# wouter-rombouts/fast-losless-image-compression-format

Measured on AMD Instinct MI355X. Metric: encode+decode MPixels/s on 4K RGBA at 1/2/4/8 MI355X; bitstream bit-exact, higher is better.
Workload: dtype u8

## Files before the change

fast-losless-image-compression-format_amd/csrc/nice_capi.hip:

```cpp
#include <hip/hip_runtime.h>
#include <stdint.h>
#include <stdio.h>
#include <stdlib.h>
#include <string.h>

#include <atomic>
#include <cmath>
#include <mutex>
#include <algorithm>
#include <vector>

#include "../../include/nice.h"
#include "../../include/nice_test.h"
#include "nice_format.h"
#include "nice_bits.hpp"
#include "nice_kernels.h"
#include "nice_dec_plan.hpp"
#include "nice_enc_plan.hpp"
#include "nice_slot_plan.hpp"
#include "nice_rec.hpp"
#include "nice_resize.hpp"
#include "nice_tiles.hpp"
#include "nice_internal.h"

// ... 400 lines not shown
  tm.end(st);
  tm.begin(NICE_PH_ENC_HEADER, st);
  hipLaunchKernelGGL(enc_header, grid_of(P.header), dim3(P.header.threads), 0, st, a);
  tm.end(st);
  if (T > 0) {
    tm.begin(NICE_PH_ENC_TILEBITS, st);
    hipLaunchKernelGGL(enc_packtab, grid_of(P.packtab), dim3(P.packtab.threads), 0, st, a);
    tm.end(st);
    launch_pack(P, a, st, &tm);
    tm.begin(NICE_PH_ENC_TAIL, st);
    hipLaunchKernelGGL(enc_tail, grid_of(P.tail), dim3(P.tail.threads), 0, st, a);
    tm.end(st);
  }
  NICE_HIP(hipGetLastError());
  return NICE_OK;
}


namespace {
struct DecLayout {
  size_t total;
  size_t o_tables, o_dstart, o_entry, o_last, o_ck, o_cpx, o_cstart, o_recs, o_changed, o_fchanged, o_rowbuf;
  size_t o_ev, o_evck, o_evn, o_agree, o_items, o_icount;
  size_t o_hand, o_abort;
};
constexpr uint32_t kSyncQueuedMax = 16, kSyncFlags = kSyncQueuedMax + 2;
constexpr uint32_t kSettledFlag = kSyncQueuedMax, kFinalFlag = kSyncQueuedMax + 1;
#ifndef NICE_SYNC_QUEUED
#define NICE_SYNC_QUEUED 8
#endif
constexpr uint32_t kSyncQueued = NICE_SYNC_QUEUED;
static_assert(kSyncQueued >= 1 && kSyncQueued <= kSyncQueuedMax, "queued sync iterations");
DecLayout dec_layout(uint32_t n_frames, uint64_t npx, const DecPlan& p) {
  const uint32_t max_chunks = p.max_chunks, n_ck = p.n_ck, ev_cap = p.ev_cap, subs = p.subs;
  DecLayout L{};
  size_t o = 0;
  auto take = [&](size_t bytes) { size_t r = o; o = align_up(o + bytes, 256); return r; };
  L.o_tables = take((size_t)n_frames * sizeof(DecTables));
  L.o_dstart = take((size_t)n_frames * 8);
  L.o_entry = take((size_t)n_frames * max_chunks * 8);
  L.o_last = take((size_t)n_frames * max_chunks * 8);
  L.o_ck = take((size_t)n_frames * n_ck * max_chunks * 8);
  L.o_cpx = take((size_t)n_frames * max_chunks * 8);
  L.o_cstart = take((size_t)n_frames * max_chunks * 8);
  L.o_recs = take((size_t)n_frames * ((npx + 3) & ~3ull) * 4);
  L.o_changed = take(4 * kSyncFlags);
  L.o_fchanged = take((size_t)n_frames * 4);
  L.o_rowbuf = take(p.rowbuf);
  L.o_ev = take((size_t)n_frames * ((max_chunks + 63) & ~63u) * ev_cap * 4);
  L.o_evck = take(ev_cap ? (size_t)n_frames * n_ck * max_chunks * 4 : 0);
  L.o_evn = take(ev_cap ? (size_t)n_frames * max_chunks * 4 : 0);
  L.o_agree = take(ev_cap ? (size_t)n_frames * max_chunks * 4 : 0);
  L.o_items = take(ev_cap ? (size_t)n_frames * max_chunks * subs * 4 : 0);
  L.o_icount = take(ev_cap ? (size_t)n_frames * 4 : 0);
  L.o_hand = take(p.hand);
  L.o_abort = take(p.abort_flags ? (size_t)n_frames * 4 : 0);
  L.total = o;
  return L;
}

void dec_args_scratch(DecArgs& a, const DecLayout& L, uint8_t* base, const DecPlan& P, uint64_t N) {
  a.tables = base + L.o_tables;
  a.data_start = (unsigned long long*)(base + L.o_dstart);
  const uint32_t max_chunks = P.max_chunks, cb = P.slice_bits;
  a.max_chunks = max_chunks;
  a.chunk_bits = cb;
  a.n_ck = P.n_ck;
  a.ck_bits = P.ck_bits;
  a.emit_blocks = (uint32_t)(((uint64_t)max_chunks * (cb / DEC_EMIT_BITS) + DEC_PARSE_THREADS - 1) / DEC_PARSE_THREADS);
  a.chunk_blocks = (max_chunks + DEC_PARSE_THREADS - 1) / DEC_PARSE_THREADS;
  a.chunk_px = (unsigned long long*)(base + L.o_cpx);
  a.chunk_start = (unsigned long long*)(base + L.o_cstart);
  a.entry = (unsigned long long*)(base + L.o_entry);
  a.last = (unsigned long long*)(base + L.o_last);
  a.ck = (unsigned long long*)(base + L.o_ck);
  a.recs = (uint32_t*)(base + L.o_recs);
  a.rec_stride = (N + 3) & ~3ull;
  a.seg = P.g.seg;
  a.nseg = P.g.nseg;
  a.rows_in_lds = P.g.in_lds ? 1u : 0u;
  a.parse_slow = opt_on(NICE_OPT_DEC_SLOW_PARSE) ? 1u : 0u;
  a.rowbuf = (uint32_t*)(base + L.o_rowbuf);
  if (P.ev_cap) {
    a.ev = (uint32_t*)(base + L.o_ev);
    a.ev_cap = P.ev_cap;
    a.ev_ck = (uint32_t*)(base + L.o_evck);
    a.ev_n = (uint32_t*)(base + L.o_evn);
    a.agree = (uint32_t*)(base + L.o_agree);
    a.head_items = (uint32_t*)(base + L.o_items);
    a.head_count = (uint32_t*)(base + L.o_icount);
  }
}

int launch_rows(const DecPlan& p, const DecLaunch& l, DecArgs& a, hipStream_t st) {
  void (*k)(DecArgs) = nullptr;
  switch (l.route) {
    case DEC_R_RECONSTRUCT: k = dec_reconstruct; break;
    case DEC_R_ROWS: k = dec_rows; break;
    case DEC_R_ROWS8: k = dec_rows8; break;
    case DEC_R_ROWS_WIDE: k = dec_rows_wide; break;
    case DEC_R_FLOW: k = dec_rows_flow; break;
    case DEC_R_SPLIT: k = dec_rows_split; break;
    default: return NICE_E_ARG;
  }
  if (l.lds > LDS_OPT_IN)
    NICE_HIP(hipFuncSetAttribute((const void*)k, hipFuncAttributeMaxDynamicSharedMemorySize, (int)l.lds));
  if (l.route != DEC_R_SPLIT) {
    hipLaunchKernelGGL(k, dim3(a.n_frames), dim3(l.threads), l.lds, st, a);
    return NICE_OK;
  }
  for (uint32_t f0 = 0; f0 < a.n_frames; f0 += p.split_frames) {
    a.split_f0 = f0;
    hipLaunchKernelGGL(k, dim3(std::min(p.split_frames, a.n_frames - f0) * p.strips), dim3(l.threads), l.lds, st, a);
// ... 14 lines not shown
          "recomputed_px=%llu fixup_rounds=%llu sync_iters=%u seg=%u nseg=%u "
          "clk[load=%llu spec=%llu fix=%llu emit=%llu]\n",
          h[0], h[1], h[2], h[3], h[4], it_count, a.seg, a.nseg, h[5], h[6], h[7], h[8]);
  fprintf(stderr, "[nice dec stats] sync iterations that changed an entry:");
  for (uint32_t i = 0; i < kSyncFlags; ++i) fprintf(stderr, " %u", chg[i]);
  fprintf(stderr, " (queued %u, then settled, final)\n", queued);
  for (int w = 0; w < 4; ++w) {
    const unsigned long long* q = h + 64 + 8 * w;
    if (q[7])
      fprintf(stderr, "[nice flow stats] wave %d rows=%llu cyc/row: emit+decode=%.0f wait=%.0f ring=%.0f spec=%.0f "
              "fix=%.0f publish=%.0f rounds/row=%.2f\n", w, q[7], (double)q[0] / q[7], (double)q[1] / q[7],
              (double)q[2] / q[7], (double)q[3] / q[7], (double)q[4] / q[7], (double)q[5] / q[7],
              (double)q[6] / q[7]);
  }
  fprintf(stderr, "[nice dec stats] unknown segment tails: copies of an unknown %llu, narrowed %llu\n", h[24], h[25]);
  fprintf(stderr, "[nice dec stats] re-parse met previous parse at checkpoint:");
  for (int k = 0; k < 17; ++k) fprintf(stderr, " %d:%llu", k, h[32 + k]);
  fprintf(stderr, "\n");
  fprintf(stderr, "[nice dec stats] slice=%u emit waves=%llu wave_iters=%llu active_lane_iters=%llu fills=%llu\n",
          a.chunk_bits, h[20], h[16], h[17], h[18]);
  fprintf(stderr, "[nice dec stats] slices by first-pass meeting checkpoint: 0:%llu 1:%llu 2-4:%llu 5-16:%llu "
          "17-64:%llu 65+:%llu none:%llu overflow:%llu (ev_cap %u)\n",
          h[50], h[51], h[52], h[53], h[54], h[55], h[56], h[57], a.ev_cap);
  fprintf(stderr, "[nice dec stats] fix-up rounds per row: 0:%llu 1:%llu 2:%llu 3:%llu 4:%llu 5:%llu 6+:%llu\n",
          h[9], h[10], h[11], h[12], h[13], h[14], h[15]);
  if (h[61]) fprintf(stderr, "[nice dec stats] sync first pass: waves=%llu cycles/wave=%.0f refill cycles/wave=%.0f "
          "refills/wave=%.1f iterations/wave=%.1f active lane share=%.3f\n",
          h[61], h[61] ? (double)h[56] / h[61] : 0.0, h[61] ? (double)h[57] / h[61] : 0.0,
          h[61] ? (double)h[58] / h[61] : 0.0, h[61] ? (double)h[59] / h[61] : 0.0,
          h[59] ? (double)h[60] / (64.0 * h[59]) : 0.0);
}
}

static std::mutex g_default_mu;
static nice_ctx* g_default = nullptr;

static int default_ctx(nice_ctx** out) {
  std::lock_guard<std::mutex> g(g_default_mu);
  if (!g_default) {
    int dev = 0;
    (void)hipGetDevice(&dev);
    int rc = nice_ctx_create(dev, &g_default);
    if (rc) return rc;
  }
  *out = g_default;
  return NICE_OK;
// ... 116 lines not shown
  NICE_HIP(hipSetDevice(ctx->device));
  hipStream_t st = (hipStream_t)stream;
  ctx->split_frames = 0;
  NICE_HIP(hipMemsetAsync(d_status, 0, (size_t)n_frames * 4, st));
  std::vector<uint64_t> lens(n_frames);
  if (h_stream_len) {
    std::copy(h_stream_len, h_stream_len + n_frames, lens.begin());
  } else {
    NICE_HIP(hipMemcpyAsync(lens.data(), d_stream_len, (size_t)n_frames * 8, hipMemcpyDeviceToHost, st));
    NICE_HIP(hipStreamSynchronize(st));
  }
  uint64_t max_len = 0;
  for (uint64_t& l : lens) {
    if (!packed && l > stream_stride) return NICE_E_ARG;
    if (packed && l > packed_bytes) l = 0;
    max_len = l > max_len ? l : max_len;
  }
  const uint64_t D = FILE_HEADER_BYTES * 8 + TABLE_HEADER_BITS;
  uint64_t total_bits = 0;
  for (uint64_t l : lens) total_bits += l * 8 > D ? l * 8 - D : 0;
  auto opt = [](int id) { return DecOpt{opt_set(id), opt_val(id)}; };
  const DecOpts opts{opt(NICE_OPT_DEC_SLICE_BITS), opt(NICE_OPT_DEC_SINGLE_WAVE), opt(NICE_OPT_DEC_SEG),
                     opt(NICE_OPT_DEC_SPLIT),      opt(NICE_OPT_DEC_FLOW),        opt(NICE_OPT_DEC_NO_EVENTS),
                     opt(NICE_OPT_DEC_EV_CAP)};
  DecPlan P = plan_decode(DecShape{n_frames, w, h, ctx->cus, max_len, total_bits}, opts);
  ctx->last_dec_route = P.rows.route;
  ctx->last_dec_fallback = P.fallback.route;
  if (N > 0 && P.rows.route == DEC_R_NONE) return NICE_E_ARG;
  DecLayout L = dec_layout(n_frames, N, P);
  int rc = ctx->dec.grow(L.total);
  if (rc && P.ev_cap) {
    (void)hipGetLastError();
    P.ev_cap = 0;
    L = dec_layout(n_frames, N, P);
    rc = ctx->dec.grow(L.total);
  }
  if (rc) return rc;
  const uint32_t max_chunks = P.max_chunks;
  uint8_t* base = (uint8_t*)ctx->dec.ptr;
  DecArgs a{};
  a.streams = d_streams;
  a.stream_stride = stream_stride;
  a.stream_len = (const unsigned long long*)d_stream_len;
  a.stream_off = (const unsigned long long*)d_stream_off;
  a.packed_bytes = packed_bytes;
  a.n_frames = n_frames;
  a.W = w;
  a.H = h;
  a.out_channels = out_channels;
  a.flags = flags;
  a.px_out = d_px;
  a.px_stride = px_stride;
  a.status = d_status;
// ... 1394 lines not shown
```

fast-losless-image-compression-format_amd/csrc/nice_dec_plan.hpp:

```cpp
#pragma once
#include <stddef.h>
#include <stdint.h>

#include "nice_format.h"
#include "nice_geom.h"

namespace nice {

struct DecShape {
  uint32_t n_frames, w, h;
  int cus;
  uint64_t max_len;
  uint64_t total_bits;
};
struct DecOpt {
  bool set;
  int64_t val;
  bool on() const { return set && val != 0; }
};
struct DecOpts { DecOpt slice_bits, single_wave, seg, split, flow, no_events, ev_cap; };

enum DecRoute : uint32_t { DEC_R_NONE, DEC_R_RECONSTRUCT, DEC_R_ROWS, DEC_R_ROWS8, DEC_R_ROWS_WIDE, DEC_R_FLOW, DEC_R_SPLIT };
constexpr uint32_t dec_route_max_threads(DecRoute r) {
  return r == DEC_R_RECONSTRUCT ? 64 : r == DEC_R_ROWS || r == DEC_R_ROWS8 ? ROWS_THREADS
       : r == DEC_R_ROWS_WIDE ? ROWS_WIDE_THREADS : r == DEC_R_FLOW ? FLOW_THREADS : r == DEC_R_SPLIT ? SPLIT_THREADS : 0;
}
struct DecLaunch {
  DecRoute route;
  uint32_t threads;
  size_t lds;
};
struct RecGeom {
  uint32_t seg, nseg, R;
  size_t lds;
  bool in_lds;
};
struct DecPlan {
  uint32_t slice_bits, max_chunks, ck_bits, n_ck, ev_cap, subs;
  DecLaunch rows;
  DecLaunch fallback;
  uint32_t strips, split_frames;
  uint32_t flow_k, flow_ring;
  size_t rowbuf, hand;
  bool abort_flags;
  RecGeom g;
};

inline RecGeom rec_geom(uint32_t w) {
  auto align4 = [](size_t v) { return (v + 3) / 4 * 4; };
  RecGeom g;
  uint32_t s = (w + DEC_MAX_SEGS - 1) / DEC_MAX_SEGS;
  if (s < 6) s = 6;
  g.seg = s;
  g.nseg = w ? (w + s - 1) / s : 1;
  if (g.nseg > 1 && w - (g.nseg - 1) * s < 6) g.nseg -= 1;
  g.R = w >= 3 ? 4 : 8;
  const size_t kw = (w + 31) / 32;
  const size_t head = 512 + align4(kw) * 4 + align4(w) * 4;
  const size_t ring = (size_t)g.R * w * 4;
  g.in_lds = head + ring <= 150 * 1024;
  g.lds = g.in_lds ? head + ring : head;
  return g;
}

inline DecPlan plan_decode(const DecShape& s, const DecOpts& o) {
  const uint32_t w = s.w, n_frames = s.n_frames;
  DecPlan p{};
  const uint64_t D = FILE_HEADER_BYTES * 8 + TABLE_HEADER_BITS;
  uint32_t cb = s.total_bits >= (48ull << 20) ? 2 * DEC_MIN_CHUNK_BITS : DEC_MIN_CHUNK_BITS;
  while (cb < DEC_MAX_CHUNK_BITS && s.total_bits / (2ull * cb) > 256ull * 8 * 64 * 2) cb *= 2;
  if (o.slice_bits.set) {
    const uint32_t v = (uint32_t)o.slice_bits.val;
    if (v >= DEC_MIN_CHUNK_BITS && v <= DEC_MAX_CHUNK_BITS && (v & (v - 1)) == 0) cb = v;
  }
  p.slice_bits = cb;
  p.max_chunks = s.max_len * 8 > D ? (uint32_t)((s.max_len * 8 - D + cb - 1) / cb) : 1;
  p.ck_bits = cb <= 4096u ? DEC_CK_BITS_SMALL : DEC_CK_BITS;
  p.n_ck = cb / p.ck_bits - 1;
  p.subs = cb / DEC_EMIT_BITS;
  p.ev_cap = o.no_events.on() ? 0u : cb / 4;
  if (o.ev_cap.set) {
    const uint32_t v = (uint32_t)o.ev_cap.val;
    if (p.ev_cap && v >= 4 && v % 4 == 0 && v < p.ev_cap) p.ev_cap = v;
  }
  const RecGeom g = p.g = rec_geom(w);
  const uint32_t cus = (uint32_t)(s.cus > 1 ? s.cus : 1);

  const uint32_t nseg16 = (w + ROWS_SEG - 1) / ROWS_SEG;
  const uint32_t rows_wpr = (nseg16 + 63) / 64, rows_thr = rows_wpr * 64;
  const bool single_wave = o.single_wave.on();
  const bool use_rows = w >= 64 && rows_thr <= ROWS_WIDE_THREADS && !single_wave;
  const size_t rows_lds = rows_lds_bytes(rows_thr, w, true);
  const bool rows_in_lds = rows_thr <= ROWS_THREADS && lds_fits(rows_lds);
  const uint32_t rows8_thr = ((w + 7) / 8 + 63) / 64 * 64;
  const size_t rows8_lds = rows_lds_bytes(rows8_thr, w, true);
  const bool rows8 = o.seg.set && o.seg.val == 8 && use_rows && rows_in_lds && rows8_thr <= ROWS_THREADS &&
                     lds_fits(rows8_lds);
  const uint32_t split_cap = (uint32_t)(s.cus / 2 > 1 ? s.cus / 2 : 1);
  uint32_t strips = (nseg16 + SPLIT_THREADS - 1) / SPLIT_THREADS;
  if (o.split.set) strips = (uint32_t)o.split.val;
  bool split = !single_wave && w >= 64 && strips >= 2 && strips <= split_cap &&
               (!use_rows || (uint64_t)n_frames * strips <= split_cap);
  if (split && !o.split.set && use_rows && w <= FLOW_MAX_W && !o.seg.on() && !(o.flow.set && o.flow.val <= 0))
    split = false;
  const uint32_t sps = split ? (nseg16 + strips - 1) / strips : 0;
  if (split && (sps > SPLIT_THREADS || nseg16 <= (strips - 1) * sps + 1)) split = false;
// ... 47 lines not shown
```

fast-losless-image-compression-format_amd/csrc/nice_decode.hip:

```cpp
#include <hip/hip_runtime.h>
#include <stdint.h>

#include <type_traits>

#include "../../include/nice.h"
#include "nice_bits.hpp"
#include "nice_dec_rec.hpp"
#include "nice_format.h"
#include "nice_kernels.h"

namespace nice {

__device__ __forceinline__ uint32_t n_chunks(uint64_t len, uint64_t D, uint32_t cb) {
  const uint64_t bits = len * 8;
  return bits > D ? (uint32_t)((bits - D + cb - 1) / cb) : 0u;
}

__global__ __launch_bounds__(256) void dec_tables(DecArgs a) {
  __shared__ uint8_t lens[N_BINS];
  __shared__ uint8_t smax[N_STREAMS];
  __shared__ uint16_t order[N_BINS];
  __shared__ int bad;
  const uint32_t f = blockIdx.x;
  const uint64_t len = a.stream_len[f];
// ... 494 lines not shown
  return c > 0xFFFFFFFFull ? 0xFFFFFFFFu : (uint32_t)c;
}
__device__ __forceinline__ uint32_t sat_add(uint32_t a, uint32_t b) { return a + b < a ? 0xFFFFFFFFu : a + b; }

constexpr unsigned long long PS_MASK = (1ull << 51) - 1ull;
__device__ __forceinline__ unsigned long long ps_pack(unsigned long long rel, uint32_t dk) {
  return rel | ((unsigned long long)dk << 44);
}


__global__ __launch_bounds__(256) void dec_init_entries(DecArgs a) {
  const uint32_t f = blockIdx.y;
  for (uint32_t j = blockIdx.x * 256 + threadIdx.x; j < a.max_chunks; j += gridDim.x * 256) {
    const uint64_t i = (uint64_t)f * a.max_chunks + j;
    a.entry[i] = ps_pack((unsigned long long)j * a.chunk_bits, 0);
    a.last[i] = ~0ull;
  }
}

__device__ __forceinline__ uint64_t ev_group(const DecArgs& a, uint32_t f, uint32_t j) {
  return ((uint64_t)f * ((a.max_chunks + 63u) & ~63u) + (j & ~63u)) * a.ev_cap + (j & 63u) * 4u;
}
__device__ __forceinline__ uint32_t ev_word(uint32_t y) { return (y >> 2) * 256u + (y & 3u); }

__device__ __forceinline__ uint32_t ev_pack(uint32_t pfx, uint32_t s0, uint32_t s1, uint32_t s2, uint32_t s3) {
  return pfx | (s0 << 3) | (s1 << 12) | (s2 << 20) | (pfx == (uint32_t)P_LUMA ? s3 << 7 : 0u);
}

__global__ __launch_bounds__(DEC_PARSE_THREADS) PARSE_ATTR void dec_sync(DecArgs a, uint32_t* changed, const uint32_t* prev,
                                                              uint32_t* fchanged) {
  __shared__ LutLds S;
  __shared__ __attribute__((aligned(16))) uint32_t ring[DEC_PARSE_THREADS * RING_STRIDE];
  if (prev && *prev == 0) return;
  const uint32_t f = blockIdx.x / a.chunk_blocks;
  const uint32_t jb = blockIdx.x % a.chunk_blocks;
  if (a.status[f] != 0) return;
  const uint64_t len = a.stream_len[f];
  const uint64_t D = a.data_start[f];
  const uint32_t nc = n_chunks(len, D, a.chunk_bits);
  if (jb * DEC_PARSE_THREADS >= nc) return;
  const uint32_t j = jb * DEC_PARSE_THREADS + threadIdx.x;
  const uint64_t base = (uint64_t)f * a.max_chunks;
  unsigned long long e = 0, last = ~0ull;
  if (j < nc) {
    e = j == 0 ? 0ull : a.entry[base + j];
    last = a.last[base + j];
  }
  const bool need = j < nc && (last == ~0ull || (last & PS_MASK) != e);
  if (!__syncthreads_or(need)) return;
  load_lut(S, reinterpret_cast<const DecTables*>(a.tables) + f);
  __syncthreads();
  const uint32_t wave = threadIdx.x >> 6;
  if (jb * DEC_PARSE_THREADS + wave * 64u >= nc) return;
  StreamParams SP;
  SP.load(S);
  uint32_t* wring = ring + wave * 64u * RING_STRIDE;
  const uint32_t* my = wring + (threadIdx.x & 63u) * RING_STRIDE;
  const uint8_t* p = dec_stream_ptr(a, f);
  const bool al16 = (reinterpret_cast<uintptr_t>(p) & 15u) == 0;
  const bool check = last != ~0ull;
  const uint32_t nvalid_old = (uint32_t)(last >> 56);
  const unsigned long long begin = D + (unsigned long long)j * a.chunk_bits;
  const unsigned long long end = begin + a.chunk_bits;
  const unsigned long long hard = len * 8 + 64;
  const uint32_t N = a.W * a.H;
  unsigned long long* ck = a.ck + (uint64_t)f * a.n_ck * a.max_chunks + j;
  const bool keep = a.ev != nullptr && !check;
  uint32_t* evp = a.ev + ev_group(a, f, j);
  uint32_t* evck = a.ev_ck + (uint64_t)f * a.n_ck * a.max_chunks + j;
  uint32_t ne = 0, ev0 = 0, ev1 = 0, ev2 = 0;
  Lane L;
  L.pos = D + (e & ((1ull << 40) - 1));
  L.rp = RING_W;
  L.ws = (uint32_t)(L.pos >> 5) - RING_W;
  uint32_t dk = (uint32_t)(e >> 44) & 127u;
  uint32_t px = 0, k = 0;
  unsigned long long next_ck = begin + a.ck_bits;
  unsigned long long ck_old = (check && nvalid_old > 0) ? ck[0] : ~0ull;
  bool active = need, synced = false;
  unsigned long long tw0 = 0, tfill = 0, nfill = 0, nit = 0, nact = 0;
#ifdef NICE_SYNC_CYCLES
  const bool tstat = a.stats != nullptr && !check;
#else
  constexpr bool tstat = false;
#endif
  if (tstat) tw0 = __builtin_amdgcn_s_memtime();
  auto parse = [&](auto fast_tag) {
    constexpr bool FAST = decltype(fast_tag)::value;
    if constexpr (FAST) {
#pragma unroll
      for (int i = 0; i < N_STREAMS; ++i) SP.g[i] = fast_param(SP.g[i]);
    }
// ... 5 lines not shown
          synced = true;
          active = false;
        } else {
          ck[(uint64_t)k * a.max_chunks] = cur | ((unsigned long long)px << 32);
          if (keep) evck[(uint64_t)k * a.max_chunks] = ne;
          ++k;
          next_ck = k < a.n_ck ? next_ck + a.ck_bits : ~0ull;
          ck_old = (check && k < nvalid_old) ? ck[(uint64_t)k * a.max_chunks] : ~0ull;
        }
      }
      if (!__any(active)) break;
      if (__any(active && !(FAST ? lane_ok_fast(L) : lane_ok(L)))) {
        const unsigned long long tf = tstat ? __builtin_amdgcn_s_memtime() : 0;
        ring_fill<FAST>(wring, p, len, al16, L);
        if (tstat) { tfill += __builtin_amdgcn_s_memtime() - tf; ++nfill; }
      }
      if (tstat) { ++nit; nact += active ? 1u : 0u; }
      if (active) {
        uint32_t s0 = 0, s1 = 0, s2 = 0, s3 = 0;
        const uint32_t pfx = FAST ? pixel_event_fast(L, my, S, SP, s0, s1, s2, s3)
                                  : pixel_event(L, my, S, SP, s0, s1, s2, s3);
        const uint32_t c = pixel_count(pfx, dk);
        px = sat_add(px, c);
        if (keep) {
          const uint32_t ev = pfx < (uint32_t)P_RUN1 ? ev_pack(pfx, s0, s1, s2, s3) : EV_RUN | min(c, EV_RUN - 1u);
          if (ne < a.ev_cap && (ne & 3u) == 3u)
            *reinterpret_cast<uint4*>(evp + ev_word(ne - 3u)) = make_uint4(ev0, ev1, ev2, ev);
          ev0 = ev1;
          ev1 = ev2;
          ev2 = ev;
          ++ne;
        }
      }
    }
  };
  const bool fast = !a.parse_slow && reinterpret_cast<const DecTables*>(a.tables)[f].fast;
  const unsigned long long B = (active && L.pos < begin ? L.pos : begin) & ~31ull;
  if (fast && __all(!active || (L.pos >= B && begin + a.chunk_bits - B < (1ull << 30)))) {
    const uint32_t fp_pfx = fast_param(SP.g[PFX_STREAM]);
    const uint32_t bwl = (uint32_t)(B >> 5);
    const uint32_t b31 = (uint32_t)(begin - B);
    const uint32_t rhard = hard > B ? (uint32_t)min(hard - B, (unsigned long long)0xFFFFFFFFu) : 0u;
    const uint32_t rlim = min(b31 + a.chunk_bits, rhard);
    uint32_t r = active ? (uint32_t)(L.pos - B) : 0u;
    uint32_t wsr = 0;
    uint32_t rfill = 0;
    uint32_t nck = b31 + a.ck_bits;
    uint32_t q0 = 0, q1 = 0, q2 = 0, q3 = 0;
    auto step = [&](auto slot_tag, auto keep_tag) -> bool {
      constexpr int SLOT = decltype(slot_tag)::value;
      constexpr bool KEEP = decltype(keep_tag)::value;
      if (active && (r >= rlim || px > N)) active = false;
      if (active && r >= nck) {
        const uint32_t cur = (r - b31) | (dk << 20);
        if (check && k < nvalid_old && (uint32_t)ck_old == cur) {
          synced = true;
          active = false;
        } else {
          ck[(uint64_t)k * a.max_chunks] = cur | ((unsigned long long)px << 32);
          if (keep) evck[(uint64_t)k * a.max_chunks] = ne;
          ++k;
          nck = k < a.n_ck ? nck + a.ck_bits : 0xFFFFFFFFu;
          ck_old = (check && k < nvalid_old) ? ck[(uint64_t)k * a.max_chunks] : ~0ull;
        }
      }
      if ((!KEEP || SLOT == 0) && !__any(active)) return false;
      if (__any(active && r >= rfill)) {
        const uint32_t wsa = (bwl + (r >> 5)) & ~3u;
        ring_fill_ws(wring, p, len, al16, wsa);
        wsr = wsa - bwl;
        rfill = (wsr + RING_W - 2u) << 5;
      }
      if (active) {
        uint32_t s0 = 0, s1 = 0, s2 = 0, s3 = 0, tot;
        const uint32_t pfx = pixel_event_fast_at(my, S, fp_pfx, (r >> 5) - wsr, r & 31u, s0, s1, s2, s3, tot);
        r += tot;
        uint32_t c;
        if (pfx < (uint32_t)P_RUN1) {
          dk = 0;
          c = 1u;
        } else {
          const uint32_t sh = (3u * dk) & 63u, d = pfx - (uint32_t)P_RUN1;
          if (sh < 30u) {
            c = (d << sh) + (dk == 0 ? 1u : 0u);
          } else {
            const uint64_t c64 = (uint64_t)d << sh;
            c = c64 > 0xFFFFFFFFull ? 0xFFFFFFFFu : (uint32_t)c64;
          }
          dk = dk >= 64u ? 1u : dk + 1u;
        }
        px = sat_add(px, c);
        if (KEEP && keep) {
          const uint32_t ev = pfx < (uint32_t)P_RUN1 ? ev_pack(pfx, s0, s1, s2, s3) : EV_RUN | min(c, EV_RUN - 1u);
          if constexpr (SLOT == 0) q0 = ev;
          if constexpr (SLOT == 1) q1 = ev;
          if constexpr (SLOT == 2) q2 = ev;
          if constexpr (SLOT == 3) {
            q3 = ev;
            if (ne < a.ev_cap) *reinterpret_cast<uint4*>(evp + ev_word(ne - 3u)) = make_uint4(q0, q1, q2, q3);
          }
          ++ne;
        }
      }
      return true;
    };
    if (__any(keep && active)) {
      for (;;) {
        if (!step(std::integral_constant<int, 0>{}, std::true_type{})) break;
        if (!step(std::integral_constant<int, 1>{}, std::true_type{})) break;
        if (!step(std::integral_constant<int, 2>{}, std::true_type{})) break;
        if (!step(std::integral_constant<int, 3>{}, std::true_type{})) break;
      }
    } else {
      while (step(std::integral_constant<int, 0>{}, std::false_type{})) {
      }
    }
    L.pos = B + r;
    const uint32_t sl = ne & 3u;
    ev0 = q0;
    ev1 = sl == 3u ? q1 : q0;
    ev2 = sl == 3u ? q2 : sl == 2u ? q1 : q0;
  } else {
    parse(std::false_type{});
  }
  if (tstat) {
    const unsigned long long tw = __builtin_amdgcn_s_memtime() - tw0;
    if ((threadIdx.x & 63u) == 0) {
      atomicAdd(&a.stats[56], tw); atomicAdd(&a.stats[57], tfill); atomicAdd(&a.stats[58], nfill);
      atomicAdd(&a.stats[59], nit); atomicAdd(&a.stats[61], 1ull);
    }
    atomicAdd(&a.stats[60], nact);
  }
  if (!need) return;
  if (keep) {
    const uint32_t slot = ne & 3u, q0 = ne & ~3u;
    if (ne <= a.ev_cap) {
      uint32_t* t = evp + ev_word(q0);
      if (slot == 3u) { t[0] = ev0; t[1] = ev1; t[2] = ev2; }
      if (slot == 2u) { t[0] = ev1; t[1] = ev2; }
      if (slot == 1u) t[0] = ev2;
    }
    a.ev_n[base + j] = ne <= a.ev_cap ? ne : EV_OVERFLOW;
    a.agree[base + j] = 0;
  } else if (a.ev) {
    const uint32_t ag = synced ? k + 1u : AGREE_NONE;
    a.agree[base + j] = max(a.agree[base + j], ag);
  }
  if (a.stats && check) {
    atomicAdd(&a.stats[32 + (synced ? min(k, 15u) : 16u)], 1ull);
  }
  if (synced) {
    const uint32_t delta = px - (uint32_t)(ck_old >> 32);
    a.chunk_px[base + j] = a.chunk_px[base + j] + (uint64_t)(int64_t)(int32_t)delta;
    for (uint32_t kk = k; kk < nvalid_old; ++kk) {
      unsigned long long& c = ck[(uint64_t)kk * a.max_chunks];
      c = (c & 0xFFFFFFFFull) | ((unsigned long long)((uint32_t)(c >> 32) + delta) << 32);
    }
    a.last[base + j] = e | ((unsigned long long)nvalid_old << 56);
    return;
  }
  a.chunk_px[base + j] = px;
  a.last[base + j] = e | ((unsigned long long)k << 56);
  if (j + 1 < nc) {
    const unsigned long long x = ps_pack(L.pos - D, dk);
    if (a.entry[base + j + 1] != x) {
      a.entry[base + j + 1] = x;
      atomicOr(changed, 1u);
      if (fchanged) fchanged[f] = 1u;
    }
// ... 335 lines not shown
  unsigned long long end = begin + a.chunk_bits;
  bool active = v < nv;
  if (active) {
    q64 = a.chunk_start[base + j];
    const uint32_t nvalid = (uint32_t)(a.last[base + j] >> 56);
    const unsigned long long* ck = a.ck + (uint64_t)f * a.n_ck * a.max_chunks + j;
    const uint32_t step = DEC_EMIT_BITS / a.ck_bits;
    if (sub == 0) {
      e = j == 0 ? 0ull : a.entry[base + j];
    } else {
      const uint32_t c = sub * step - 1;
      if (c < nvalid) {
        const unsigned long long x = ck[(uint64_t)c * a.max_chunks];
        e = ((begin - D) + (x & 0xFFFFu)) | ((unsigned long long)((x >> 20) & 127u) << 44);
        q64 += x >> 32;
      } else {
        active = false;
      }
    }
    const uint32_t c1 = (sub + 1) * step - 1;
    if (sub + 1 < subs && c1 < nvalid) end = begin + (ck[(uint64_t)c1 * a.max_chunks] & 0xFFFFu);
    if (q64 > N) active = false;
    if (a.ev) {
      const uint32_t ag = a.agree[base + j];
      if (ag != AGREE_NONE && a.ev_n[base + j] != EV_OVERFLOW && ag <= nvalid) {
        const unsigned long long stop =
            ag == 0u ? begin : begin + (ck[(uint64_t)(ag - 1u) * a.max_chunks] & 0xFFFFu);
        if (stop < end) end = stop;
        if (sub * step >= ag) active = false;
      }
    }
  }
  uint32_t q = (uint32_t)(q64 > N ? N : q64);
  const uint32_t q0 = q;
  const unsigned long long hard = len * 8 + 64;
  uint32_t* rec = a.recs + (uint64_t)f * a.rec_stride;
  const bool strict = (a.flags & NICE_DEC_STRICT_REFERENCE) != 0;
  Lane L;
  L.pos = D + (e & ((1ull << 40) - 1));
  L.rp = RING_W;
  L.ws = (uint32_t)(L.pos >> 5) - RING_W;
  uint32_t dk = (uint32_t)(e >> 44) & 127u;
  bool closed = (q == N);
  bool err = false;
  RecGroup G{~0ull, REC_RUN, REC_RUN, REC_RUN, REC_RUN, 0u};
  auto handle = [&](bool at_n, uint32_t pfx, uint32_t s0, uint32_t s1, uint32_t s2, uint32_t s3) {
    if (at_n) {
      if (dk != 0 && pfx == (uint32_t)P_RUN1) { (void)pixel_count(pfx, dk); return; }
      err = err || (strict && pfx >= (uint32_t)P_RUN1);
      active = false;
// ... 62 lines not shown
      r += tot;
      handle(at_n, pfx, s0, s1, s2, s3);
    }
  } else {
    emit(std::false_type{});
  }
  G.flush(rec, q0, q0);
  if (err) set_status(&a.status[f], NICE_E_FORMAT);
}

__global__ __launch_bounds__(1024) void dec_heads(DecArgs a) {
  __shared__ uint32_t part[1024];
  const uint32_t f = blockIdx.x;
  if (a.status[f] != 0) {
    if (threadIdx.x == 0) a.head_count[f] = 0;
    return;
  }
  const uint32_t nc = n_chunks(a.stream_len[f], a.data_start[f], a.chunk_bits);
  const uint64_t base = (uint64_t)f * a.max_chunks;
  const uint32_t subs = a.chunk_bits / DEC_EMIT_BITS, step = DEC_EMIT_BITS / a.ck_bits;
  const uint32_t per = (nc + 1023) / 1024;
  const uint32_t c0 = min(threadIdx.x * per, nc), c1 = min(c0 + per, nc);
  auto nsub = [&](uint32_t j) -> uint32_t {
    const uint32_t ag = a.agree[base + j], nvalid = (uint32_t)(a.last[base + j] >> 56);
    if (ag == AGREE_NONE || a.ev_n[base + j] == EV_OVERFLOW || ag > nvalid)
      return min(subs, 1u + nvalid / step);
    return (ag + step - 1) / step;
  };
  uint32_t cnt = 0;
  for (uint32_t j = c0; j < c1; ++j) cnt += nsub(j);
  part[threadIdx.x] = cnt;
  __syncthreads();
  for (uint32_t d = 1; d < 1024; d <<= 1) {
    const uint32_t t = threadIdx.x >= d ? part[threadIdx.x - d] : 0u;
    __syncthreads();
    part[threadIdx.x] += t;
    __syncthreads();
  }
  uint32_t o = part[threadIdx.x] - cnt;
  uint32_t* items = a.head_items + base * subs;
  for (uint32_t j = c0; j < c1; ++j) {
    const uint32_t n = nsub(j);
    for (uint32_t s = 0; s < n; ++s) items[o++] = j * subs + s;
  }
  if (threadIdx.x == 1023) a.head_count[f] = part[1023];
}

__device__ __forceinline__ uint32_t place_record(uint32_t ev, uint32_t q, uint32_t W, const uint32_t* sdl,
                                                 const uint2* idt, bool& bad) {
// ... 29 lines not shown
    const uint32_t rd = i % 7u, t1 = i / 7u;
    t.v[i] = ((rd - 3u) & 255u) | ((((t1 % 7u) - 3u) & 255u) << 10) | ((((t1 / 7u) - 3u) & 255u) << 20);
  }
  return t;
}
__device__ __constant__ SdlTable kSdl = make_sdl_table();

__global__ __launch_bounds__(64 * DEC_PLACE_WAVES) void dec_place(DecArgs a) {
  __shared__ __attribute__((aligned(16))) uint32_t sdl[344];
  __shared__ uint2 idt[16];
  if (threadIdx.x < 16u) {
    const uint32_t id = threadIdx.x;
    const uint32_t cls = (uint32_t)(ID_CLS_PACK >> (4u * id)) & 15u;
    idt[id] = make_uint2(cls, (uint32_t)((CLS_ROWS_PACK >> (2u * cls)) & 3u) * a.W +
                                  (uint32_t)((CLS_PX_PACK >> (3u * cls)) & 7u));
  }
  if (threadIdx.x < 86u)
    reinterpret_cast<uint4*>(sdl)[threadIdx.x] = reinterpret_cast<const uint4*>(kSdl.v)[threadIdx.x];
  __syncthreads();
  const uint32_t lane = threadIdx.x & 63u;
  const uint32_t nbx = gridDim.x, nwg = nbx * gridDim.y, lin = blockIdx.y * nbx + blockIdx.x;
  const uint32_t xq = nwg / 8u, xr = nwg % 8u, xcd = lin % 8u;
  const uint32_t lg = (xcd < xr ? xcd * (xq + 1u) : xr * (xq + 1u) + (xcd - xr) * xq) + lin / 8u;
  const uint32_t f = lg / nbx, j = (lg % nbx) * DEC_PLACE_WAVES + (threadIdx.x >> 6);
  if (a.status[f] != 0) return;
  const uint64_t len = a.stream_len[f];
  const uint64_t D = a.data_start[f];
  if (j >= n_chunks(len, D, a.chunk_bits)) return;
  const uint64_t base = (uint64_t)f * a.max_chunks;
  const uint32_t ag = a.agree[base + j], nev = a.ev_n[base + j];
  const uint32_t nvalid = (uint32_t)(a.last[base + j] >> 56);
  if (a.stats && lane == 0) {
    const uint32_t b = nev == EV_OVERFLOW ? 7u : ag == AGREE_NONE ? 6u : ag == 0u ? 0u : ag == 1u ? 1u
                     : ag <= 4u ? 2u : ag <= 16u ? 3u : ag <= 64u ? 4u : 5u;
    atomicAdd(&a.stats[50 + b], 1ull);
  }
  if (ag == AGREE_NONE || nev == EV_OVERFLOW || ag > nvalid) return;
  const uint64_t cki = (uint64_t)f * a.n_ck * a.max_chunks + j + (uint64_t)(ag ? ag - 1u : 0u) * a.max_chunks;
  const uint32_t i_first = ag == 0u ? 0u : a.ev_ck[cki];
  unsigned long long q = a.chunk_start[base + j] + (ag == 0u ? 0ull : (a.ck[cki] >> 32));
  const uint64_t N = (uint64_t)a.W * a.H;
  if (q > N) return;
  const uint32_t* evp = a.ev + ev_group(a, f, j);
  uint32_t* rec = a.recs + (uint64_t)f * a.rec_stride;
  const bool strict = (a.flags & NICE_DEC_STRICT_REFERENCE) != 0;
  bool err = false;
  if (i_first >= nev) return;
  const uint32_t ev_last = nev - 1u;
  uint32_t nx[4];
#pragma unroll
  for (int k = 0; k < 4; ++k) nx[k] = evp[ev_word(min(i_first + 64u * k + lane, ev_last))];
  for (uint32_t i = i_first; i < nev; i += 256u) {
    uint32_t ev[4], r[4];
#pragma unroll
    for (int k = 0; k < 4; ++k) {
      ev[k] = nx[k];
      nx[k] = evp[ev_word(min(i + 256u + 64u * k + lane, ev_last))];
    }
    {
      const uint32_t N32 = (uint32_t)N;
      uint32_t c32[4];
      bool big = false;
#pragma unroll
      for (int k = 0; k < 4; ++k) {
        const bool valid = i + 64u * k + lane < nev;
        c32[k] = valid ? ((ev[k] & EV_RUN) ? (ev[k] & ~EV_RUN) : 1u) : 0u;
        big = big || c32[k] >= 65536u;
      }
      if (!__any(big)) {
        uint32_t qb[4];
// ... 44 lines not shown
      }
      const unsigned long long qb = q + carry + incl - c[k];
      carry += __shfl(incl, 63);
      qk[k] = qb;
      bool rbad = false;
      r[k] = place_record(ev[k], (uint32_t)min(qb, N), a.W, sdl, idt, rbad);
      const bool at_n = valid && qb == N && !(run && c[k] == 0);
      const bool bad = valid && !at_n && (run ? qb + c[k] > N : rbad);
      const unsigned long long m = __ballot(at_n || bad);
      if (stop_k == 4u && m) {
        stop_k = (uint32_t)k;
        stop_lane = (uint32_t)__builtin_ctzll(m);
        stop_at_n = __shfl(at_n ? 1 : 0, (int)stop_lane) != 0;
        stop_run = __shfl(run ? 1 : 0, (int)stop_lane) != 0;
      }
    }
#pragma unroll
    for (int k = 0; k < 4; ++k) {
      const bool keep = (uint32_t)k < stop_k || ((uint32_t)k == stop_k && lane < stop_lane);
      if (keep && i + 64u * k + lane < nev && !(ev[k] & EV_RUN)) rec[qk[k]] = r[k] | rec_tagbits(a.rec_tag);
    }
    if (stop_k < 4u) {
      if (lane == 0) err = stop_at_n ? (strict && stop_run) : true;
      break;
    }
    q += carry;
  }
  if (err) set_status(&a.status[f], NICE_E_FORMAT);
}


}
```

fast-losless-image-compression-format_amd/csrc/nice_kernels.h:

```cpp
#pragma once
#include <hip/hip_runtime.h>
#include <stdint.h>

#include "nice_geom.h"

namespace nice {

constexpr uint32_t FLAG_LONG = 1u;
constexpr uint32_t FLAG_BAD = 2u;

struct EncArgs {
  const uint8_t* px;
  uint64_t frame_stride;
  uint32_t n_frames, W, H, C;
  uint8_t channels_out;
  uint32_t tiles_per_frame, tiles_per_block;
  uint8_t* out;
  uint64_t out_stride;
  unsigned long long* out_len;
  uint32_t* hist;
  uint32_t* tile_first;
  uint32_t* tile_last;
  uint32_t* tile_next;
  uint32_t* cmask;
// ... 95 lines not shown
  unsigned long long* entry;
  unsigned long long* last;
  unsigned long long* ck;
  uint32_t chunk_bits, n_ck;
  uint32_t ck_bits;
  uint32_t emit_blocks;
  unsigned long long* chunk_px;
  unsigned long long* chunk_start;
  uint32_t* recs;
  uint64_t rec_stride;
  uint32_t seg, nseg;
  uint32_t rows_in_lds;
  uint32_t rec_tag;
  uint32_t parse_slow;
  uint32_t* rowbuf;
  unsigned long long* stats;
  uint32_t* ev;
  uint32_t ev_cap;
  uint32_t* ev_ck;
  uint32_t* ev_n;
  uint32_t* agree;
  uint32_t* head_items;
  uint32_t* head_count;
  uint32_t strips;
  unsigned long long* hand;
  uint32_t* hand_abort;
  uint32_t split_f0;
  uint32_t redo;
  uint32_t test_absent_strip;
  uint32_t flow_k, flow_ring;
  const uint32_t* unsettled;
  const unsigned long long* stream_off;
  uint64_t packed_bytes;
};
__device__ __forceinline__ const uint8_t* dec_stream_ptr(const DecArgs& a, uint32_t f) {
  return a.streams + (a.stream_off ? (uint64_t)a.stream_off[f] : (uint64_t)f * a.stream_stride);
}
constexpr uint32_t SPLIT_ABORT_ERR = 1u, SPLIT_REDO = 2u;
constexpr uint32_t EV_RUN = 1u << 31, EV_BAD = 1u << 9, EV_L2 = 1u << 8;
constexpr uint32_t EV_OVERFLOW = 0xFFFFFFFFu, AGREE_NONE = 0xFFFFu;

__global__ void dec_tables(DecArgs a);
__global__ void dec_init_entries(DecArgs a);
__global__ void dec_sync(DecArgs a, uint32_t* changed, const uint32_t* prev, uint32_t* fchanged);
__global__ void dec_sync_settle(DecArgs a, const uint32_t* last_changed, const uint32_t* fchanged, uint32_t* settled);
__global__ void dec_scan(DecArgs a);
// ... 30 lines not shown
```

Before: 68180.

## Record re-parse events for slice heads so placement replaces head emission

During the checkpoint re-parse (check pass), the decoder now stores the pixel events it sees for a slice's head into a new per-slice head-event buffer (hev), sized from the checkpoint spacing. The placement kernel can then place the head events and continue with the first-pass events once the meeting checkpoint matches. This lets the emit kernels skip slices whose head was captured, avoiding a second parse of the head region. It adds scratch memory, extra stores in the re-parse loop, an extra template branch, and a consistency check that flags an error if the head's end does not land on the meeting position.

```diff
diff --git a/fast-losless-image-compression-format_amd/csrc/nice_capi.hip b/fast-losless-image-compression-format_amd/csrc/nice_capi.hip
--- a/fast-losless-image-compression-format_amd/csrc/nice_capi.hip
+++ b/fast-losless-image-compression-format_amd/csrc/nice_capi.hip
@@ -446,6 +446,7 @@
   size_t total;
   size_t o_tables, o_dstart, o_entry, o_last, o_ck, o_cpx, o_cstart, o_recs, o_changed, o_fchanged, o_rowbuf;
   size_t o_ev, o_evck, o_evn, o_agree, o_items, o_icount;
+  size_t o_hev, o_hevn, o_hevag;
   size_t o_hand, o_abort;
 };
 constexpr uint32_t kSyncQueuedMax = 16, kSyncFlags = kSyncQueuedMax + 2;
@@ -477,6 +478,10 @@
   L.o_agree = take(ev_cap ? (size_t)n_frames * max_chunks * 4 : 0);
   L.o_items = take(ev_cap ? (size_t)n_frames * max_chunks * subs * 4 : 0);
   L.o_icount = take(ev_cap ? (size_t)n_frames * 4 : 0);
+  const uint32_t hev_cap = ev_cap ? p.hev_cap : 0u;
+  L.o_hev = take((size_t)n_frames * ((max_chunks + 63) & ~63u) * hev_cap * 4);
+  L.o_hevn = take(hev_cap ? (size_t)n_frames * max_chunks * 4 : 0);
+  L.o_hevag = take(hev_cap ? (size_t)n_frames * max_chunks * 4 : 0);
   L.o_hand = take(p.hand);
   L.o_abort = take(p.abort_flags ? (size_t)n_frames * 4 : 0);
   L.total = o;
@@ -513,6 +518,12 @@
     a.agree = (uint32_t*)(base + L.o_agree);
     a.head_items = (uint32_t*)(base + L.o_items);
     a.head_count = (uint32_t*)(base + L.o_icount);
+    if (P.hev_cap) {
+      a.hev = (uint32_t*)(base + L.o_hev);
+      a.hev_cap = P.hev_cap;
+      a.hev_n = (uint32_t*)(base + L.o_hevn);
+      a.hev_ag = (uint32_t*)(base + L.o_hevag);
+    }
   }
 }
 
@@ -573,6 +584,8 @@
   fprintf(stderr, "[nice dec stats] slices by first-pass meeting checkpoint: 0:%llu 1:%llu 2-4:%llu 5-16:%llu "
           "17-64:%llu 65+:%llu none:%llu overflow:%llu (ev_cap %u)\n",
           h[50], h[51], h[52], h[53], h[54], h[55], h[56], h[57], a.ev_cap);
+  fprintf(stderr, "[nice dec stats] slice heads: none=%llu placed=%llu emitted=%llu whole_slice_emitted=%llu "
+          "invariant_violations=%llu (hev_cap %u)\n", h[26], h[27], h[28], h[29], h[30], a.hev_cap);
   fprintf(stderr, "[nice dec stats] fix-up rounds per row: 0:%llu 1:%llu 2:%llu 3:%llu 4:%llu 5:%llu 6+:%llu\n",
           h[9], h[10], h[11], h[12], h[13], h[14], h[15]);
   if (h[61]) fprintf(stderr, "[nice dec stats] sync first pass: waves=%llu cycles/wave=%.0f refill cycles/wave=%.0f "
@@ -735,13 +748,19 @@
   auto opt = [](int id) { return DecOpt{opt_set(id), opt_val(id)}; };
   const DecOpts opts{opt(NICE_OPT_DEC_SLICE_BITS), opt(NICE_OPT_DEC_SINGLE_WAVE), opt(NICE_OPT_DEC_SEG),
                      opt(NICE_OPT_DEC_SPLIT),      opt(NICE_OPT_DEC_FLOW),        opt(NICE_OPT_DEC_NO_EVENTS),
-                     opt(NICE_OPT_DEC_EV_CAP)};
+                     opt(NICE_OPT_DEC_EV_CAP),     opt(NICE_OPT_DEC_HEV_CAP)};
   DecPlan P = plan_decode(DecShape{n_frames, w, h, ctx->cus, max_len, total_bits}, opts);
   ctx->last_dec_route = P.rows.route;
   ctx->last_dec_fallback = P.fallback.route;
   if (N > 0 && P.rows.route == DEC_R_NONE) return NICE_E_ARG;
   DecLayout L = dec_layout(n_frames, N, P);
   int rc = ctx->dec.grow(L.total);
+  if (rc && P.hev_cap) {
+    (void)hipGetLastError();
+    P.hev_cap = 0;
+    L = dec_layout(n_frames, N, P);
+    rc = ctx->dec.grow(L.total);
+  }
   if (rc && P.ev_cap) {
     (void)hipGetLastError();
     P.ev_cap = 0;
diff --git a/fast-losless-image-compression-format_amd/csrc/nice_dec_plan.hpp b/fast-losless-image-compression-format_amd/csrc/nice_dec_plan.hpp
--- a/fast-losless-image-compression-format_amd/csrc/nice_dec_plan.hpp
+++ b/fast-losless-image-compression-format_amd/csrc/nice_dec_plan.hpp
@@ -18,7 +18,7 @@
   int64_t val;
   bool on() const { return set && val != 0; }
 };
-struct DecOpts { DecOpt slice_bits, single_wave, seg, split, flow, no_events, ev_cap; };
+struct DecOpts { DecOpt slice_bits, single_wave, seg, split, flow, no_events, ev_cap, hev_cap; };
 
 enum DecRoute : uint32_t { DEC_R_NONE, DEC_R_RECONSTRUCT, DEC_R_ROWS, DEC_R_ROWS8, DEC_R_ROWS_WIDE, DEC_R_FLOW, DEC_R_SPLIT };
 constexpr uint32_t dec_route_max_threads(DecRoute r) {
@@ -37,6 +37,7 @@
 };
 struct DecPlan {
   uint32_t slice_bits, max_chunks, ck_bits, n_ck, ev_cap, subs;
+  uint32_t hev_cap;
   DecLaunch rows;
   DecLaunch fallback;
   uint32_t strips, split_frames;
@@ -82,6 +83,14 @@
   if (o.ev_cap.set) {
     const uint32_t v = (uint32_t)o.ev_cap.val;
     if (p.ev_cap && v >= 4 && v % 4 == 0 && v < p.ev_cap) p.ev_cap = v;
+  }
+  {
+    const uint32_t head_bits = 2 * p.ck_bits < cb ? 2 * p.ck_bits : cb;
+    p.hev_cap = p.ev_cap ? (head_bits / 4 + 3u) & ~3u : 0u;
+  }
+  if (o.hev_cap.set) {
+    const uint32_t v = (uint32_t)o.hev_cap.val;
+    if (p.hev_cap && v >= 4 && v % 4 == 0 && v < p.hev_cap) p.hev_cap = v;
   }
   const RecGeom g = p.g = rec_geom(w);
   const uint32_t cus = (uint32_t)(s.cus > 1 ? s.cus : 1);
diff --git a/fast-losless-image-compression-format_amd/csrc/nice_decode.hip b/fast-losless-image-compression-format_amd/csrc/nice_decode.hip
--- a/fast-losless-image-compression-format_amd/csrc/nice_decode.hip
+++ b/fast-losless-image-compression-format_amd/csrc/nice_decode.hip
@@ -540,6 +540,31 @@
   return ((uint64_t)f * ((a.max_chunks + 63u) & ~63u) + (j & ~63u)) * a.ev_cap + (j & 63u) * 4u;
 }
 __device__ __forceinline__ uint32_t ev_word(uint32_t y) { return (y >> 2) * 256u + (y & 3u); }
+__device__ __forceinline__ uint64_t hev_group(const DecArgs& a, uint32_t f, uint32_t j) {
+  return ((uint64_t)f * ((a.max_chunks + 63u) & ~63u) + (j & ~63u)) * a.hev_cap + (j & 63u) * 4u;
+}
+
+constexpr uint32_t SLICE_EMIT = 0, SLICE_HEAD_EMIT = 1, SLICE_PLACE = 2;
+__device__ __forceinline__ uint32_t slice_route(const DecArgs& a, uint64_t base, uint32_t j, uint32_t& ag,
+                                                uint32_t& nvalid, uint32_t& hn) {
+  const unsigned long long last = a.last[base + j];
+  ag = a.agree[base + j];
+  const uint32_t nev = a.ev_n[base + j];
+  unsigned long long e = 0;
+  uint32_t hev_n = EV_OVERFLOW, hev_ag = AGREE_NONE;
+  if (a.hev) {
+    e = j == 0 ? 0ull : a.entry[base + j];
+    hev_n = a.hev_n[base + j];
+    hev_ag = a.hev_ag[base + j];
+  }
+  nvalid = (uint32_t)(last >> 56);
+  hn = 0;
+  if (ag == AGREE_NONE || nev == EV_OVERFLOW || ag > nvalid) return SLICE_EMIT;
+  if (ag == 0u) return SLICE_PLACE;
+  if ((last & PS_MASK) != e || hev_n == EV_OVERFLOW || hev_ag != ag) return SLICE_HEAD_EMIT;
+  hn = hev_n;
+  return SLICE_PLACE;
+}
 
 __device__ __forceinline__ uint32_t ev_pack(uint32_t pfx, uint32_t s0, uint32_t s1, uint32_t s2, uint32_t s3) {
   return pfx | (s0 << 3) | (s1 << 12) | (s2 << 20) | (pfx == (uint32_t)P_LUMA ? s3 << 7 : 0u);
@@ -584,8 +609,10 @@
   const uint32_t N = a.W * a.H;
   unsigned long long* ck = a.ck + (uint64_t)f * a.n_ck * a.max_chunks + j;
   const bool keep = a.ev != nullptr && !check;
-  uint32_t* evp = a.ev + ev_group(a, f, j);
+  uint32_t* evp = check ? a.hev + hev_group(a, f, j) : a.ev + ev_group(a, f, j);
   uint32_t* evck = a.ev_ck + (uint64_t)f * a.n_ck * a.max_chunks + j;
+  const bool hkeep = a.hev != nullptr && check && need;
+  bool hkept = false;
   uint32_t ne = 0, ev0 = 0, ev1 = 0, ev2 = 0;
   Lane L;
   L.pos = D + (e & ((1ull << 40) - 1));
@@ -637,9 +664,9 @@
                                   : pixel_event(L, my, S, SP, s0, s1, s2, s3);
         const uint32_t c = pixel_count(pfx, dk);
         px = sat_add(px, c);
-        if (keep) {
+        if (keep || hkeep) {
           const uint32_t ev = pfx < (uint32_t)P_RUN1 ? ev_pack(pfx, s0, s1, s2, s3) : EV_RUN | min(c, EV_RUN - 1u);
-          if (ne < a.ev_cap && (ne & 3u) == 3u)
+          if (ne < (keep ? a.ev_cap : a.hev_cap) && (ne & 3u) == 3u)
             *reinterpret_cast<uint4*>(evp + ev_word(ne - 3u)) = make_uint4(ev0, ev1, ev2, ev);
           ev0 = ev1;
           ev1 = ev2;
@@ -664,7 +691,8 @@
     uint32_t q0 = 0, q1 = 0, q2 = 0, q3 = 0;
     auto step = [&](auto slot_tag, auto keep_tag) -> bool {
       constexpr int SLOT = decltype(slot_tag)::value;
-      constexpr bool KEEP = decltype(keep_tag)::value;
+      constexpr bool KEEP = decltype(keep_tag)::value == 1;
+      constexpr bool HEAD = decltype(keep_tag)::value == 2;
       if (active && (r >= rlim || px > N)) active = false;
       if (active && r >= nck) {
         const uint32_t cur = (r - b31) | (dk << 20);
@@ -679,7 +707,7 @@
           ck_old = (check && k < nvalid_old) ? ck[(uint64_t)k * a.max_chunks] : ~0ull;
         }
       }
-      if ((!KEEP || SLOT == 0) && !__any(active)) return false;
+      if ((!(KEEP || HEAD) || SLOT == 0) && !__any(active)) return false;
       if (__any(active && r >= rfill)) {
         const uint32_t wsa = (bwl + (r >> 5)) & ~3u;
         ring_fill_ws(wring, p, len, al16, wsa);
@@ -716,18 +744,40 @@
           }
           ++ne;
         }
+        if (HEAD && hkeep) {
+          const uint32_t ev = pfx < (uint32_t)P_RUN1 ? ev_pack(pfx, s0, s1, s2, s3) : EV_RUN | min(c, EV_RUN - 1u);
+          if constexpr (SLOT == 0) q0 = ev;
+          if constexpr (SLOT == 1) q1 = ev;
+          if constexpr (SLOT == 2) q2 = ev;
+          if constexpr (SLOT == 3) {
+            q3 = ev;
+            if (ne < a.hev_cap) *reinterpret_cast<uint4*>(evp + ev_word(ne - 3u)) = make_uint4(q0, q1, q2, q3);
+          }
+          ++ne;
+        }
       }
       return true;
     };
+    using keep_none = std::integral_constant<int, 0>;
+    using keep_first = std::integral_constant<int, 1>;
+    using keep_head = std::integral_constant<int, 2>;
     if (__any(keep && active)) {
       for (;;) {
-        if (!step(std::integral_constant<int, 0>{}, std::true_type{})) break;
-        if (!step(std::integral_constant<int, 1>{}, std::true_type{})) break;
-        if (!step(std::integral_constant<int, 2>{}, std::true_type{})) break;
-        if (!step(std::integral_constant<int, 3>{}, std::true_type{})) break;
+        if (!step(std::integral_constant<int, 0>{}, keep_first{})) break;
+        if (!step(std::integral_constant<int, 1>{}, keep_first{})) break;
+        if (!step(std::integral_constant<int, 2>{}, keep_first{})) break;
+        if (!step(std::integral_constant<int, 3>{}, keep_first{})) break;
+      }
+    } else if (__any(hkeep && active)) {
+      hkept = true;
+      for (;;) {
+        if (!step(std::integral_constant<int, 0>{}, keep_head{})) break;
+        if (!step(std::integral_constant<int, 1>{}, keep_head{})) break;
+        if (!step(std::integral_constant<int, 2>{}, keep_head{})) break;
+        if (!step(std::integral_constant<int, 3>{}, keep_head{})) break;
       }
     } else {
-      while (step(std::integral_constant<int, 0>{}, std::false_type{})) {
+      while (step(std::integral_constant<int, 0>{}, keep_none{})) {
       }
     }
     L.pos = B + r;
@@ -737,6 +787,7 @@
     ev2 = sl == 3u ? q2 : sl == 2u ? q1 : q0;
   } else {
     parse(std::false_type{});
+    hkept = true;
   }
   if (tstat) {
     const unsigned long long tw = __builtin_amdgcn_s_memtime() - tw0;
@@ -747,19 +798,25 @@
     atomicAdd(&a.stats[60], nact);
   }
   if (!need) return;
+  auto store_tail = [&](uint32_t* t) {
+    const uint32_t slot = ne & 3u;
+    if (slot == 3u) { t[0] = ev0; t[1] = ev1; t[2] = ev2; }
+    if (slot == 2u) { t[0] = ev1; t[1] = ev2; }
+    if (slot == 1u) t[0] = ev2;
+  };
   if (keep) {
-    const uint32_t slot = ne & 3u, q0 = ne & ~3u;
-    if (ne <= a.ev_cap) {
-      uint32_t* t = evp + ev_word(q0);
-      if (slot == 3u) { t[0] = ev0; t[1] = ev1; t[2] = ev2; }
-      if (slot == 2u) { t[0] = ev1; t[1] = ev2; }
-      if (slot == 1u) t[0] = ev2;
-    }
+    if (ne <= a.ev_cap) store_tail(evp + ev_word(ne & ~3u));
     a.ev_n[base + j] = ne <= a.ev_cap ? ne : EV_OVERFLOW;
     a.agree[base + j] = 0;
   } else if (a.ev) {
     const uint32_t ag = synced ? k + 1u : AGREE_NONE;
     a.agree[base + j] = max(a.agree[base + j], ag);
+    if (a.hev) {
+      const bool ok = synced && hkept && ne <= a.hev_cap;
+      if (ok) store_tail(evp + ev_word(ne & ~3u));
+      a.hev_n[base + j] = ok ? ne : EV_OVERFLOW;
+      a.hev_ag[base + j] = ag;
+    }
   }
   if (a.stats && check) {
     atomicAdd(&a.stats[32 + (synced ? min(k, 15u) : 16u)], 1ull);
@@ -1141,10 +1198,11 @@
     if (sub + 1 < subs && c1 < nvalid) end = begin + (ck[(uint64_t)c1 * a.max_chunks] & 0xFFFFu);
     if (q64 > N) active = false;
     if (a.ev) {
-      const uint32_t ag = a.agree[base + j];
-      if (ag != AGREE_NONE && a.ev_n[base + j] != EV_OVERFLOW && ag <= nvalid) {
-        const unsigned long long stop =
-            ag == 0u ? begin : begin + (ck[(uint64_t)(ag - 1u) * a.max_chunks] & 0xFFFFu);
+      uint32_t ag, nv2, hn;
+      const uint32_t route = slice_route(a, base, j, ag, nv2, hn);
+      if (route == SLICE_PLACE) active = false;
+      if (route == SLICE_HEAD_EMIT) {
+        const unsigned long long stop = begin + (ck[(uint64_t)(ag - 1u) * a.max_chunks] & 0xFFFFu);
         if (stop < end) end = stop;
         if (sub * step >= ag) active = false;
       }
@@ -1253,9 +1311,10 @@
   const uint32_t per = (nc + 1023) / 1024;
   const uint32_t c0 = min(threadIdx.x * per, nc), c1 = min(c0 + per, nc);
   auto nsub = [&](uint32_t j) -> uint32_t {
-    const uint32_t ag = a.agree[base + j], nvalid = (uint32_t)(a.last[base + j] >> 56);
-    if (ag == AGREE_NONE || a.ev_n[base + j] == EV_OVERFLOW || ag > nvalid)
-      return min(subs, 1u + nvalid / step);
+    uint32_t ag, nvalid, hn;
+    const uint32_t route = slice_route(a, base, j, ag, nvalid, hn);
+    if (route == SLICE_EMIT) return min(subs, 1u + nvalid / step);
+    if (route == SLICE_PLACE) return 0u;
     return (ag + step - 1) / step;
   };
   uint32_t cnt = 0;
@@ -1331,30 +1390,47 @@
   const uint32_t nbx = gridDim.x, nwg = nbx * gridDim.y, lin = blockIdx.y * nbx + blockIdx.x;
   const uint32_t xq = nwg / 8u, xr = nwg % 8u, xcd = lin % 8u;
   const uint32_t lg = (xcd < xr ? xcd * (xq + 1u) : xr * (xq + 1u) + (xcd - xr) * xq) + lin / 8u;
-  const uint32_t f = lg / nbx, j = (lg % nbx) * DEC_PLACE_WAVES + (threadIdx.x >> 6);
+  const uint32_t f = lg / nbx, j = (lg % nbx) * DEC_PLACE_WAVES + (uint32_t)__builtin_amdgcn_readfirstlane((int)(threadIdx.x >> 6));
   if (a.status[f] != 0) return;
   const uint64_t len = a.stream_len[f];
   const uint64_t D = a.data_start[f];
   if (j >= n_chunks(len, D, a.chunk_bits)) return;
   const uint64_t base = (uint64_t)f * a.max_chunks;
-  const uint32_t ag = a.agree[base + j], nev = a.ev_n[base + j];
-  const uint32_t nvalid = (uint32_t)(a.last[base + j] >> 56);
+  uint32_t ag, nvalid, hn;
+  const uint32_t route = slice_route(a, base, j, ag, nvalid, hn);
+  const uint32_t nev = a.ev_n[base + j];
   if (a.stats && lane == 0) {
     const uint32_t b = nev == EV_OVERFLOW ? 7u : ag == AGREE_NONE ? 6u : ag == 0u ? 0u : ag == 1u ? 1u
                      : ag <= 4u ? 2u : ag <= 16u ? 3u : ag <= 64u ? 4u : 5u;
     atomicAdd(&a.stats[50 + b], 1ull);
-  }
-  if (ag == AGREE_NONE || nev == EV_OVERFLOW || ag > nvalid) return;
+    atomicAdd(&a.stats[route == SLICE_EMIT ? 29 : route == SLICE_HEAD_EMIT ? 28 : ag == 0u ? 26 : 27], 1ull);
+  }
+  if (route == SLICE_EMIT) return;
+  const bool head = route == SLICE_PLACE && ag != 0u;
   const uint64_t cki = (uint64_t)f * a.n_ck * a.max_chunks + j + (uint64_t)(ag ? ag - 1u : 0u) * a.max_chunks;
-  const uint32_t i_first = ag == 0u ? 0u : a.ev_ck[cki];
-  unsigned long long q = a.chunk_start[base + j] + (ag == 0u ? 0ull : (a.ck[cki] >> 32));
+  auto uni = [](uint32_t v) { return (uint32_t)__builtin_amdgcn_readfirstlane((int)v); };
+  const uint32_t i_first1 = uni(ag == 0u ? 0u : a.ev_ck[cki]), nev1 = uni(nev);
+  hn = uni(hn);
+  const unsigned long long q_first = a.chunk_start[base + j];
+  const unsigned long long q_meet_v = q_first + (ag == 0u ? 0ull : (a.ck[cki] >> 32));
+  const unsigned long long q_meet = ((unsigned long long)uni((uint32_t)(q_meet_v >> 32)) << 32) | uni((uint32_t)q_meet_v);
+  unsigned long long q = head ? q_first : q_meet;
   const uint64_t N = (uint64_t)a.W * a.H;
   if (q > N) return;
-  const uint32_t* evp = a.ev + ev_group(a, f, j);
   uint32_t* rec = a.recs + (uint64_t)f * a.rec_stride;
   const bool strict = (a.flags & NICE_DEC_STRICT_REFERENCE) != 0;
-  bool err = false;
-  if (i_first >= nev) return;
+  bool err = false, stopped = false;
+  for (uint32_t part = head ? 0u : 1u; part < 2u && !stopped; ++part) {
+  const uint32_t* evp = part == 0u ? a.hev + hev_group(a, f, j) : a.ev + ev_group(a, f, j);
+  const uint32_t i_first = part == 0u ? 0u : i_first1, nev = part == 0u ? hn : nev1;
+  if (part == 1u && head && q != q_meet) {
+    if (lane == 0) {
+      if (a.stats) atomicAdd(&a.stats[30], 1ull);
+      set_status(&a.status[f], NICE_E_HIP);
+    }
+    return;
+  }
+  if (i_first >= nev) continue;
   const uint32_t ev_last = nev - 1u;
   uint32_t nx[4];
 #pragma unroll
@@ -1445,10 +1521,12 @@
     }
     if (stop_k < 4u) {
       if (lane == 0) err = stop_at_n ? (strict && stop_run) : true;
+      stopped = true;
       break;
     }
     q += carry;
   }
+  }
   if (err) set_status(&a.status[f], NICE_E_FORMAT);
 }
 
diff --git a/fast-losless-image-compression-format_amd/csrc/nice_kernels.h b/fast-losless-image-compression-format_amd/csrc/nice_kernels.h
--- a/fast-losless-image-compression-format_amd/csrc/nice_kernels.h
+++ b/fast-losless-image-compression-format_amd/csrc/nice_kernels.h
@@ -141,6 +141,10 @@
   uint32_t* agree;
   uint32_t* head_items;
   uint32_t* head_count;
+  uint32_t* hev;
+  uint32_t hev_cap;
+  uint32_t* hev_n;
+  uint32_t* hev_ag;
   uint32_t strips;
   unsigned long long* hand;
   uint32_t* hand_abort;
```

Result: faster. 69060 (median of 6 runs) (+1.3%).
